# max-andr/joint-cnn-mrf

Hardware: AMD Instinct MI355X
Metric: images/sec (720x480, K=9 joints) part-detector+spatial-model fwd (higher is better)
Workload: dtype f32(fp16x2 spectra, fft); 1 GPU; configs[1]: batch=64/GPU synthetic 480x720x3, part detector + spatial model forward + argmax, fp32; batch_per_gpu=64, global_batch=64, micro_batch=64, use_sm=True, collective=all_gather coords int32 [B,2,9]

## Files before the change

joint-cnn-mrf_amd/csrc/conv_fft.hip:

```cpp
#include <cmath>
#include <cstdlib>
#include <map>
#include <mutex>
#include <utility>
#include <vector>

#include "conv_fft_common.h"

namespace jcm {
namespace cfft {

template <int KS, int NP>
__global__ __launch_bounds__(256) void weight_spectra_split_kernel(const float* __restrict__ w, uint4* __restrict__ Ws, int Cin, int Cout, int CoutP, int ntl, int NY, int NX,
                                                                   int round_bf16, float* __restrict__ wscale) {
  __shared__ cf twy[192][KS - 1], twx[KS];
  const int tid = threadIdx.x;
  const int kx = blockIdx.y;
#pragma unroll 1
  for (int k = tid; k < NY * (KS - 1) + KS; k += 256) {
    const bool isy = k < NY * (KS - 1);
    const int ky = k / (KS - 1), a = isy ? k % (KS - 1) + 1 : k - NY * (KS - 1);
    const int num = isy ? (ky * a) % NY : (kx * a) % NX, den = isy ? NY : NX;
    double sn, cs;
    sincospi(-2.0 * (double)num / (double)den, &sn, &cs);
// ... 115 lines not shown
  }
  block_max_to<256>(m * 1.0001f, wmax, red, threadIdx.x);
}

struct Sizes { int NY, NX; };
static const int kLens[] = {20, 24, 28, 32, 36, 40, 50, 60, 64, 72, 96, 100, 128, 192};
static bool pick(int need, int* n) {
  for (int v : kLens)
    if (v >= need) { *n = v; return true; }
  return false;
}
static int tw_offset(int n) {
  int off = 0;
  for (int v : kLens) {
    if (v == n) return off;
    off += v;
  }
  return -1;
}
static bool sizes_of(int H, int W, int ks, Sizes* s, int circ = 0) {
  if (circ) {
    s->NY = H; s->NX = W;
    return (ks == 9 || ks == 5) && H > 8 && W > 8 && tw_offset(H) >= 0 && tw_offset(W) >= 0;
  }
  return (ks == 9 || ks == 5) && H + ks - 1 <= 192 && W + ks - 1 <= 192 && pick(H + 4, &s->NY) && pick(W + 4, &s->NX);
}
static int pad64(int c) { return (c + CB - 1) / CB * CB; }
static bool fft_reg_on() {
  static const bool on = [] { const char* e = std::getenv("JCM_FFT_REG"); return !e || std::atoi(e) != 0; }();
  return on;
}
static bool fft_tiles_on() {
  static const bool on = [] { const char* e = std::getenv("JCM_FFT_TILES"); return !e || std::atoi(e) != 0; }();
  return on;
}
static int padn(int c, int n) { return (c + n - 1) / n * n; }

int persistent_grid(const void* kernel, int ntiles, int threads, int dyn_lds) {
  static std::mutex mu;
  static std::map<std::pair<const void*, int>, int> cache;
  int dev = 0;
  (void)hipGetDevice(&dev);
  int resident = 0;
  {
    std::lock_guard<std::mutex> lk(mu);
    auto it = cache.find({kernel, dev});
    if (it != cache.end()) resident = it->second;
  }
  if (!resident) {
    int ncu = 256, per_cu = 0;
    (void)hipDeviceGetAttribute(&ncu, hipDeviceAttributeMultiprocessorCount, dev);
    if (hipOccupancyMaxActiveBlocksPerMultiprocessor(&per_cu, kernel, threads, (size_t)dyn_lds) != hipSuccess || per_cu < 1) per_cu = 1;
    resident = ncu * per_cu;
    std::lock_guard<std::mutex> lk(mu);
    cache[{kernel, dev}] = resident;
  }
  return resident < ntiles ? resident : ntiles;
}

static const cf* twiddle_table(int dev) {
  static std::mutex mu;
  static std::map<int, cf*> tabs;
  std::lock_guard<std::mutex> lk(mu);
  auto it = tabs.find(dev);
  if (it != tabs.end()) return it->second;
  std::vector<float> h;
// ... 201 lines not shown
    }
    if (hipError_t ce = cfft_cols_fwd(s.NY, a, np, Tin, Xs, twy, p.NXH, p.MT, sc, st); ce != hipSuccess) return ce;
  }
  if (hipError_t e = hipGetLastError(); e != hipSuccess) return e;
  if (g0 && hipEventRecord(g0, st) != hipSuccess) return hipErrorUnknown;
  const float yshift = sc.t16 ? cgemm_split_y16_shift(a.Cin) : 0.f, yinv = yshift != 0.f ? 1.0f / yshift : 0.f;
  if (hipError_t e = cgemm_split(Xs, a.wp, Yf, np, p.F, a.B, a.Cin, a.Cout, p.ldy, st, yshift); e != hipSuccess) return e;
  if (g1 && hipEventRecord(g1, st) != hipSuccess) return hipErrorUnknown;
  ConvArgs ai = a;
  if (a0.circ) { ai.H = a0.H - 8; ai.W = a0.W - 8; }
  if (!(fft_reg && p.inv_cb == 64 && cfft_cols_inv_reg(s.NY, ai, Yf, T, p.NXH, p.ldy, opad, st, sc.t16_inv, yinv))) cfft_cols_inv(s.NY, ai, Yf, T, twy, p.NXH, p.ldy, opad, st, sc.t16_inv, yinv);
  if (t_next && nx && nx->pool) {
    Sizes sn;
    if (!sizes_of((a.H + 1) / 2, (a.W + 1) / 2, nx->ks_next, &sn) ||
        !cfft_rows_inv_pool_fwd(s.NX, sn.NX, a, T, static_cast<cf*>(t_next), twx, twb + tw_offset(sn.NX), opad, norm, sc, st))
      return hipErrorInvalidValue;
  } else if (t_next && nx && nx->merge) {
    if (sc.t16) {
      float* t16n = reinterpret_cast<float*>(static_cast<char*>(t_next) + align256((size_t)a.B * p.NXH * a.H * a.Cout * 4));
      if (!(fft_reg && cfft_rows_inv_merge_fwd_reg(s.NX, a, *nx->merge, T, static_cast<cf*>(t_next), opad, norm, sc, st, t16n))) return hipErrorInvalidValue;
    } else if (!(fft_reg && cfft_rows_inv_merge_fwd_reg(s.NX, a, *nx->merge, T, static_cast<cf*>(t_next), opad, norm, sc, st)) &&
               !cfft_rows_inv_merge_fwd(s.NX, a, *nx->merge, T, static_cast<cf*>(t_next), twx, opad, norm, sc, st)) {
      return hipErrorInvalidValue;
    }
  } else if (t_next) {
    if (!(fft_reg && cfft_rows_inv_fwd_reg(s.NX, a, T, static_cast<cf*>(t_next), opad, norm, sc, st))) cfft_rows_inv_fwd(s.NX, a, T, static_cast<cf*>(t_next), twx, opad, norm, sc, st);
  } else if (!((ai.rows_mfma & 1) && cfft_rows_inv_mfma(s.NX, ai, out_layout, T, opad, norm, sc, st)) && !(fft_reg && cfft_rows_inv_reg(s.NX, ai, out_layout, T, opad, norm, sc, st))) {
    if (ai.wout_TX > 0) return hipErrorInvalidValue;
    cfft_rows_inv(s.NX, ai, out_layout, T, twx, opad, norm, sc, st);
  }
  return hipGetLastError();
}

size_t conv_fft_xs_bytes(const ConvArgs& a, int ks, int np) {
  Sizes s;
  if (!sizes_of(a.H, a.W, ks, &s, a.circ)) return 0;
  return align256(plan_of(a, s, np).xs_bytes);
}
hipError_t conv_fft_spectra(const ConvArgs& a0, int ks, int np, void* work, void* xs, hipStream_t st, float* tmax, int common) {
  Sizes s;
  if (!conv_fft_supported(a0, ks) || !sizes_of(a0.H, a0.W, ks, &s, a0.circ) || !xs || (np >= 4 && !tmax)) return hipErrorInvalidValue;
  Fp16Scale sc;
  if (np >= 4) { sc.tmax = tmax; sc.hf = (float)a0.H; sc.nb = a0.B; sc.common = common; }
  ConvArgs a = a0;
  a.CoutP = pad64(a.Cout);
  const Plan3 p = plan_of(a, s, np);
  int dev = 0;
  if (hipError_t e = hipGetDevice(&dev); e != hipSuccess) return e;
  const cf* twb = twiddle_table(dev);
  if (!twb) return hipErrorOutOfMemory;
  cf* T = static_cast<cf*>(work);
  if (a.win_map) { if (!cfft_rows_fwd_win_reg(s.NX, a, T, sc.tmax, st)) return hipErrorInvalidValue; }
  else cfft_rows_fwd(s.NX, a, 0, T, twb + tw_offset(s.NX), sc.tmax, st);
  if (hipError_t ce = cfft_cols_fwd(s.NY, a, np, T, xs, twb + tw_offset(s.NY), p.NXH, p.MT, sc, st); ce != hipSuccess) return ce;
  return hipGetLastError();
}
bool conv_fft_geometry(int H, int W, int ks, int B, int Cout, int np, int* NY, int* NX, int* MT, int circ) {
  Sizes s;
  if (!sizes_of(H, W, ks, &s, circ)) return false;
  *NY = s.NY; *NX = s.NX; *MT = cgemm_split_mtile(np, B, Cout);
  return true;
}

}
```

joint-cnn-mrf_amd/csrc/conv_fft_common.h:

```cpp
#pragma once
#include "fft_lds.h"
#include "kernels.h"

namespace jcm {
namespace cfft {
using namespace fftl;
constexpr int CB = 64, NT = 256;
constexpr int kParMax = 512;

template <int N> struct Plan;
template <> struct Plan<192> { static constexpr int R1 = 8, R2 = 8, R3 = 3; };
template <> struct Plan<128> { static constexpr int R1 = 8, R2 = 4, R3 = 4; };
template <> struct Plan<100> { static constexpr int R1 = 4, R2 = 5, R3 = 5; };
template <> struct Plan<96> { static constexpr int R1 = 8, R2 = 12, R3 = 1; };
template <> struct Plan<72> { static constexpr int R1 = 8, R2 = 3, R3 = 3; };
template <> struct Plan<64> { static constexpr int R1 = 8, R2 = 8, R3 = 1; };
template <> struct Plan<60> { static constexpr int R1 = 4, R2 = 15, R3 = 1; };
template <> struct Plan<50> { static constexpr int R1 = 5, R2 = 10, R3 = 1; };
template <> struct Plan<40> { static constexpr int R1 = 8, R2 = 5, R3 = 1; };
template <> struct Plan<36> { static constexpr int R1 = 4, R2 = 3, R3 = 3; };
template <> struct Plan<32> { static constexpr int R1 = 8, R2 = 4, R3 = 1; };
template <> struct Plan<28> { static constexpr int R1 = 4, R2 = 7, R3 = 1; };
template <> struct Plan<24> { static constexpr int R1 = 8, R2 = 3, R3 = 1; };
template <> struct Plan<20> { static constexpr int R1 = 4, R2 = 5, R3 = 1; };
// ... 225 lines not shown
    case 64: CALL(64); break;                    \
    case 72: CALL(72); break;                    \
    case 96: CALL(96); break;                    \
    case 100: CALL(100); break;                  \
    case 128: CALL(128); break;                  \
    default: CALL(192); break;                   \
  }

int persistent_grid(const void* kernel, int ntiles, int threads, int dyn_lds = 0);

void cfft_rows_fwd(int NX, const ConvArgs& a, int layout, cf* T, const cf* tw, float* tmax, hipStream_t st, float* t16 = nullptr);
void cfft_rows_fwd_merge(int NX, const ConvArgs& a, const FftMerge& m, int in_layout, cf* T, const cf* tw, float* tmax, hipStream_t st, float* t16 = nullptr);
hipError_t cfft_cols_fwd(int NY, const ConvArgs& a, int np, const cf* T, void* Xs, const cf* tw, int NXH, int MT, const Fp16Scale& sc, hipStream_t st);
void cfft_cols_inv(int NY, const ConvArgs& a, const cf* Yf, cf* T, const cf* tw, int NXH, int ldy, int pad, hipStream_t st, float* t16 = nullptr, float y16_inv = 0.f);
void cfft_rows_inv(int NX, const ConvArgs& a, int layout, const cf* T, const cf* tw, int pad, float norm, const Fp16Scale& sc, hipStream_t st);
bool cfft_rows_inv_reg(int NX, const ConvArgs& a, int layout, const cf* T, int pad, float norm, const Fp16Scale& sc, hipStream_t st);
bool cfft_rows_inv_fwd_reg(int NX, const ConvArgs& a, const cf* T, cf* Tn, int pad, float norm, const Fp16Scale& sc, hipStream_t st);
bool cfft_rows_fwd_reg(int NX, const ConvArgs& a, int layout, cf* T, float* tmax, hipStream_t st, float* t16);
bool cfft_rows_fwd_win_reg(int NX, const ConvArgs& a, cf* T, float* tmax, hipStream_t st);
bool cfft_rows_fwd_win_reg_supported(int NX, int Cin);
bool cfft_tiles_supported(int NY, int NX, const ConvArgs& a);
bool cfft_rows_fwd_tile_reg(int NY, int NX, const ConvArgs& a, cf* T, float* tmax, hipStream_t st);
bool cfft_rows_inv_pool_tile_reg(int NY, int NX, const ConvArgs& a, const cf* T, cf* Tn, float norm, const Fp16Scale& sc, hipStream_t st);
bool cfft_rows_fwd_merge_reg(int NX, const ConvArgs& a, const FftMerge& m, int in_layout, cf* T, float* tmax, hipStream_t st, float* t16);
bool cfft_cols_inv_reg(int NY, const ConvArgs& a, const cf* Yf, cf* T, int NXH, int ldy, int pad, hipStream_t st, float* t16, float y16_inv = 0.f);
void cfft_rows_inv_fwd(int NX, const ConvArgs& a, const cf* T, cf* Tn, const cf* tw, int pad, float norm, const Fp16Scale& sc, hipStream_t st);
bool cfft_rows_inv_pool_fwd(int NXI, int NXO, const ConvArgs& a, const cf* T, cf* Tn, const cf* twi, const cf* two, int pad, float norm, const Fp16Scale& sc, hipStream_t st);
bool cfft_rows_inv_merge_fwd(int NX, const ConvArgs& a, const FftMerge& m, const cf* T, cf* Tn, const cf* tw, int pad, float norm, const Fp16Scale& sc, hipStream_t st);
bool cfft_rows_inv_merge_fwd_reg(int NX, const ConvArgs& a, const FftMerge& m, const cf* T, cf* Tn, int pad, float norm, const Fp16Scale& sc, hipStream_t st, float* t16n = nullptr);
bool cfft_rows_inv_merge_fwd_reg_supported(int NX, const ConvArgs& a, const FftMerge& m, int pad);
bool cfft_rows_inv_pool_fwd_supported(int NXI, int NXO, int Cout);
bool cfft_rows_inv_mfma(int NX, const ConvArgs& a, int layout, const cf* T, int pad, float norm, const Fp16Scale& sc, hipStream_t st);
bool cfft_rows_inv_merge_fwd_supported(int NX, const ConvArgs& a, const FftMerge& m);
}
}
```

joint-cnn-mrf_amd/csrc/ctx.h:

```cpp
#pragma once
#include "../../include/jcm.h"

#include <map>
#include <mutex>
#include <string>
#include <vector>

#include "kernels.h"

namespace jcm {

struct CallOrder;

int fail(int code, const std::string& msg);

#define HIP_TRY(expr)                                                                                   \
  do {                                                                                                  \
    hipError_t e_ = (expr);                                                                             \
    if (e_ != hipSuccess)                                                                               \
      return ::jcm::fail(JCM_ERR_HIP, std::string(#expr) + ": " + hipGetErrorString(e_));               \
  } while (0)
#define JCM_TRY(expr)          \
  do {                         \
    int r_ = (expr);           \
// ... 27 lines not shown
  void* wp_kxfold = nullptr;
  void* wq1_bf16 = nullptr;
  float* wq1_f32 = nullptr;
  void* wq1_split = nullptr;
  int coutp_bf16 = 0;
  bool thin = false;
  bool thin_bf16 = false;
  const float* bias = nullptr;
  float* scale = nullptr;
  float* shift = nullptr;
};

struct TrainState;
}
struct jcm_ctx;
namespace jcm {
void train_destroy(jcm_ctx* c);
const float* train_param_range(jcm_ctx* c, int64_t off, int64_t n);
const double* train_grad_sumsq(jcm_ctx* c);

}

struct jcm_ctx {
  int device = 0;
  hipStream_t stream = nullptr;
  int precision = JCM_PRECISION_F32;
  int K = 9;
  bool finalized = false;
  int f32_conv = 0;
  int split_min_wgs = 128;
  int sm_algo = 3;
  int conv9_fft = 1;
  int fft_tiles = 1;
  int fft_fuse = 3;
  int fft_single = 1;
  int fft_t16 = 1;
  int fft_rows_mfma = 1;
  int fft_win = 1;
  int bf16_hpool = 1;
  int sm_chunk = 32;
  int micro_batch = 0;
  int call_order = 1;
  int debug_skip = 0;
  std::map<std::string, jcm::Tensor> params;
  std::map<std::string, jcm::ConvLayer> convs;
  std::vector<void*> owned;
  size_t param_bytes = 0;
  bool has_sm = false;
  float* sp_energy = nullptr;
  float* sp_bias = nullptr;
  float* bn_sm_scale = nullptr;
  float* bn_sm_shift = nullptr;
  int* cond = nullptr;
  const float** energy_ptrs = nullptr;
  const float** bias_ptrs = nullptr;
  int* cond0 = nullptr;
  float2* prior_spec_t = nullptr;
  struct FftW { void* p = nullptr; size_t bytes = 0; bool valid = false; float* wscale = nullptr; };
  std::map<std::string, FftW> fft_w;
  double* hist_limits = nullptr;
  jcm::TrainState* train = nullptr;
  char* arena = nullptr;
  size_t arena_cap = 0, arena_off = 0, arena_peak = 0;
  bool dry = false;
  float* act_scale = nullptr;
  float* scale_scratch = nullptr;
// ... 87 lines not shown
```

joint-cnn-mrf_amd/csrc/jcm_api.hip:

```cpp
#include <cmath>
#include <cstdlib>
#include <cstdio>
#include <cstring>

#include <mutex>
#include <vector>

#include "ctx.h"

using namespace jcm;

namespace {
thread_local std::string g_err;
}

namespace jcm {

const char* const kJointNames[10] = {"lsho", "lelb", "lwri", "rsho", "relb", "rwri", "lhip", "rhip", "nose", "torso"};

int fail(int code, const std::string& msg) {
  g_err = msg;
  return code;
}

// ... 219 lines not shown
      jcm_ctx::WordBlock& b = c->fft_blocks[c->fft_block_i];
      if (c->fft_word_i + n <= b.cap) {
        *w = b.p + c->fft_word_i;
        c->fft_word_i += n;
        return JCM_OK;
      }
      ++c->fft_block_i;
      c->fft_word_i = 0;
      continue;
    }
    jcm_ctx::WordBlock b;
    b.cap = n > jcm_ctx::kFftWords ? n : jcm_ctx::kFftWords;
    HIP_TRY(hipMalloc(reinterpret_cast<void**>(&b.p), (size_t)b.cap * sizeof(float)));
    if (hipError_t e = hipMemsetAsync(b.p, 0, (size_t)b.cap * sizeof(float), c->stream); e != hipSuccess) {
      (void)hipFree(b.p);
      return fail(JCM_ERR_HIP, std::string("hipMemsetAsync: ") + hipGetErrorString(e));
    }
    c->fft_blocks.push_back(b);
  }
}
int run_conv_fft(jcm_ctx* c, const ConvLayer* L, const std::string& scope, const void* x, int B, int H, int W, void* out, int in_layout, int out_layout, int circ, FftLink* link) {
  FftLink alone;
  FftLink& k = link ? *link : alone;
  ConvArgs a{};
  a.x = x; a.bias = L->bias; a.scale = L->scale; a.shift = L->shift; a.out = out;
  a.B = B; a.H = H; a.W = W; a.Cin = L->cin; a.Cout = L->cout; a.CoutP = L->cout; a.relu_bn = L->has_bn ? 1 : 0;
  a.circ = circ;
  a.rows_mfma = c->fft_rows_mfma;
  const size_t mark = c->arena_off;
  const int np = fft_np(c);
  a.tiles = c->fft_tiles && k.next.pool && !k.t_in && !k.xs && !k.merge && !k.win_map && !circ && in_layout == 0 &&
            np == 4 && conv_fft_tiles_supported(a, L->ks, k.next.ks_next) ? 1 : 0;
  const int wH = a.tiles ? H / 2 : H, wW = a.tiles ? W / 2 : W;
  void* work = arena_alloc<char>(c, conv_fft_workspace_bytes(a, L->ks, np));
  c->arena_off = mark;
  if (c->dry) return JCM_OK;
  const std::string key = scope + (circ ? "@win" : "@") + std::to_string(wH) + "x" + std::to_string(wW);
  if (!c->fft_w.count(key)) {
    static const size_t cap = [] { const char* e = std::getenv("JCM_FFT_CACHE_GB"); return (size_t)(e ? std::atoi(e) : 64) << 30; }();
    const size_t need = conv_fft_weight_bytes(wH, wW, L->ks, L->cin, L->cout, np, circ);
    size_t held = 0;
    for (auto& kv : c->fft_w) held += kv.second.bytes;
    if (held + need > cap && !c->fft_w.empty()) {
      HIP_TRY(hipStreamSynchronize(c->stream));
      for (auto& kv : c->fft_w) (void)hipFree(kv.second.p);
      c->fft_w.clear();
    }
  }
  jcm_ctx::FftW& fw = c->fft_w[key];
  if (!fw.p) {
    const size_t wb = (conv_fft_weight_bytes(wH, wW, L->ks, L->cin, L->cout, np, circ) + 255) & ~size_t(255);
    fw.bytes = wb + 256;
    if (hipMalloc(&fw.p, fw.bytes) == hipSuccess) {
      fw.wscale = reinterpret_cast<float*>(static_cast<char*>(fw.p) + wb);
    } else {
      const size_t mb = fw.bytes >> 20;
      c->fft_w.erase(key);
      return fail(JCM_ERR_HIP, "out of device memory for the filter spectra of '" + scope + "' (" + std::to_string(mb) + " MB); jcm_set_option(\"conv9_fft\", 0) selects the direct kernels");
    }
  }
  if (!fw.valid) {
    const float* bound_from = nullptr;
    if (np >= 4 && scope.compare(0, 6, "dgrad:") == 0) {
      auto it = c->fft_w.find(key.substr(6));
      if (it != c->fft_w.end() && it->second.valid && it->second.wscale) bound_from = it->second.wscale;
    }
    HIP_TRY(conv_fft_pack_weights(L->w_raw, fw.p, wH, wW, L->ks, L->cin, L->cout, np, c->precision == JCM_PRECISION_BF16, c->stream, fw.wscale, circ, bound_from));
    fw.valid = true;
  }
  a.wp = fw.p;
  hipEvent_t e0 = nullptr, e1 = nullptr, g0 = nullptr, g1 = nullptr;
  JCM_TRY(prof_begin(c, &e0, &e1));
  if (c->profile && (pool_get(c, &g0) != JCM_OK || pool_get(c, &g1) != JCM_OK)) { g0 = g1 = nullptr; }
  if (k.win_map) {
    a.win_map = k.win_map; a.win_B = k.win_B; a.win_H = k.win_H; a.win_W = k.win_W; a.win_TY = k.win_TY; a.win_TX = k.win_TX;
  }
  if (k.win_scatter) {
    a.wout_H = k.win_H; a.wout_W = k.win_W; a.wout_TY = k.win_TY; a.wout_TX = k.win_TX;
  }
  Fp16Scale sc;
  if (np >= 4) {
    sc.tmax = k.tmax_in;
    if ((k.t_in || k.xs_ready) && !sc.tmax) return fail(JCM_ERR_STATE, "conv_fft '" + scope + "': a handed-over tensor without its scale word");
    if (!sc.tmax) JCM_TRY(fft_new_words(c, a.tiles ? 4 * B : B, &sc.tmax));
    if (k.t_next) JCM_TRY(fft_new_words(c, B, &sc.tmax_next));
    sc.winv = fw.wscale + 1;
    sc.common = c->train ? 1 : 0;
    sc.t16 = (np == 5 && c->fft_t16 && in_layout != 0 && out_layout != 0 && !k.xs && (!k.t_in || k.t_in_16) && (!k.t_next || (k.next.merge && !k.t_in))) ? 1 : 0;
  }
  k.tmax = sc.tmax;
  k.tmax_next = sc.tmax_next;
  const hipError_t e = conv_fft_f32(a, L->ks, np, in_layout, out_layout, work, k, g0, g1, c->stream, np >= 4 ? &sc : nullptr);
  if (g0 && g1 && e == hipSuccess) c->prof[scope + "/gemm"].emplace_back(g0, g1);
  else { if (g0) c->event_pool.push_back(g0); if (g1) c->event_pool.push_back(g1); }
  prof_end(c, scope, e0, e1, e == hipSuccess);
  if (e != hipSuccess) return fail(JCM_ERR_HIP, std::string("conv_fft_f32: ") + hipGetErrorString(e));
  return JCM_OK;
}

int run_conv_layer(jcm_ctx* c, const ConvLayer* L, const std::string& scope, int stride, const void* x, int B, int H, int W, int sub,
                   void* out, bool act_bf16, bool out_f32, int in_planar, int out_planar, bool x_u8, FftLink* link, int hpool) {
  const bool fft = stride == 1 && takes_fft(c, L, B, H, W);
  if (!fft && link && !link->empty()) return fail(JCM_ERR_STATE, "layer '" + scope + "' was given a frequency-domain hand-over but does not run in the frequency domain");
  if (hpool && (fft || stride != 1)) return fail(JCM_ERR_STATE, "half pool requested for layer '" + scope + "', which does not run on conv5_strip_bf16_kernel");
  if (stride == 2) {
    if (c->dry) return JCM_OK;
    if (!(L->ks == 5 && L->cin == 3 && L->has_bn))
      return fail(JCM_ERR_ARG, "stride-2 kernel exists for 5x5, Cin=3, BN layers only (" + scope + ")");
    HIP_TRY(conv1_5x5s2(x, L->w_raw, L->bias, L->scale, L->shift, out, act_bf16, B, H, W, sub, L->cout, c->stream, x_u8));
    return JCM_OK;
  }
  if (fft) return run_conv_fft(c, L, scope, x, B, H, W, out, act_bf16 ? (in_planar ? 2 : 1) : 0, (act_bf16 && !out_f32) ? (out_planar ? 2 : 1) : 0, 0, link);
  if (c->dry) return JCM_OK;
  const void* wp = act_bf16 ? L->wp_bf16 : static_cast<const void*>(L->wp);
  if (stride != 1 || !wp) return fail(JCM_ERR_ARG, "no kernel for layer '" + scope + "' with stride " + std::to_string(stride));
  if (!act_bf16 && L->wp_stale) {
    HIP_TRY(pack_weights_f32(L->w_raw, L->wp, L->ks, L->cin, L->cout, L->coutp, c->stream));
    L->wp_stale = false;
  }
  hipEvent_t e0 = nullptr, e1 = nullptr;
  JCM_TRY(prof_begin(c, &e0, &e1));
  const int r = launch_conv_layer(c, L, wp, x, B, H, W, out, act_bf16, out_f32, in_planar, out_planar, hpool);
  prof_end(c, scope, e0, e1, r == JCM_OK);
  return r;
}
// ... 385 lines not shown
  }
  if (k == "debug_skip") {
    h->debug_skip = (int)value;
    return JCM_OK;
  }
  if (k == "call_order") {
    h->call_order = value != 0;
    return JCM_OK;
  }
  if (k == "conv9_fft") {
    h->conv9_fft = value != 0;
    return JCM_OK;
  }
  if (k == "fft_single") {
    if ((value != 0) != (h->fft_single != 0)) {
      HIP_TRY(hipStreamSynchronize(h->stream));
      for (auto& kv : h->fft_w) (void)hipFree(kv.second.p);
      h->fft_w.clear();
    }
    h->fft_single = value != 0;
    return JCM_OK;
  }
  if (k == "fft_windows") {
    h->fft_win = value != 0;
    return JCM_OK;
  }
  if (k == "fft_fuse") {
    if (value < 0 || value > 3) return fail(JCM_ERR_ARG, "fft_fuse must be 0..3 (bit 0: pool hand-over, bit 1: merge hand-over)");
    h->fft_fuse = (int)value;
    return JCM_OK;
  }
  if (k == "fft_tiles") {
    h->fft_tiles = value != 0;
    return JCM_OK;
  }
  if (k == "bf16_hpool") {
    h->bf16_hpool = value != 0;
    return JCM_OK;
  }
  if (k == "fft_rows_mfma") {
    h->fft_rows_mfma = value != 0;
    return JCM_OK;
  }
  if (k == "fft_t16") {
    h->fft_t16 = value != 0;
    return JCM_OK;
  }
  if (k == "sm_chunk") {
    if (value < 1) return fail(JCM_ERR_ARG, "sm_chunk must be >= 1");
    h->sm_chunk = (int)value;
    return JCM_OK;
  }
  if (k == "split_min_wgs") {
    if (value < 0) return fail(JCM_ERR_ARG, "split_min_wgs must be >= 0");
    h->split_min_wgs = (int)value;
    return JCM_OK;
  }
  if (k == "sm_algo") {
    if (value != 1 && value != 3) return fail(JCM_ERR_ARG, "sm_algo must be 3 (every transform in LDS, default) or 1 (direct sliding-window kernel); the rocFFT routes 0 and 2 were removed in round 5");
    h->sm_algo = (int)value;
    return JCM_OK;
  }
  if (h->finalized) return fail(JCM_ERR_STATE, "options must be set before jcm_finalize");
  if (k == "precision") {
    if (value != JCM_PRECISION_F32 && value != JCM_PRECISION_BF16) return fail(JCM_ERR_ARG, "precision must be 0 (f32) or 1 (bf16)");
    h->precision = (int)value;
// ... 479 lines not shown
```

joint-cnn-mrf_amd/csrc/kernels.h:

```cpp
#pragma once
#include <hip/hip_runtime.h>
#include <stdint.h>

#include <atomic>

namespace jcm {

struct LdsAttr {
  std::atomic<uint64_t> done{0};
  hipError_t ensure(const void* fn, int bytes) {
    int dev = 0;
    hipError_t e = hipGetDevice(&dev);
    if (e != hipSuccess) return e;
    const uint64_t bit = 1ull << (dev & 63);
    if (done.load(std::memory_order_acquire) & bit) return hipSuccess;
    e = hipFuncSetAttribute(fn, hipFuncAttributeMaxDynamicSharedMemorySize, bytes);
    if (e == hipSuccess) done.fetch_or(bit, std::memory_order_release);
    return e;
  }
};

struct ConvArgs {
  const void* x;
  const void* wp;
// ... 38 lines not shown
  int nb = 0;
  int common = 0;
  int t16 = 0;
  float* t16_fwd = nullptr;
  float* t16_inv = nullptr;
  int t16_cb = 64;
};
bool conv_fft_supported(const ConvArgs& a, int ks);
size_t conv_fft_weight_bytes(int H, int W, int ks, int Cin, int Cout, int np, int circ = 0);
hipError_t conv_fft_pack_weights(const float* w_hwio, void* wf, int H, int W, int ks, int Cin, int Cout, int np, bool round_bf16, hipStream_t st,
                                 float* wscale = nullptr, int circ = 0,
                                 const float* bound_from = nullptr);
size_t conv_fft_workspace_bytes(const ConvArgs& a, int ks, int np);
struct FftMerge { const void* x2; int H2, W2; const void* x3; int H3, W3; };
struct FftNext { int pool = 0; int ks_next = 0; const FftMerge* merge = nullptr; };
struct FftLink {
  const void* t_in = nullptr;
  bool t_in_16 = false;
  float* tmax_in = nullptr;
  const FftMerge* merge = nullptr;
  void* xs = nullptr;
  bool xs_ready = false;
  const void* win_map = nullptr;
  int win_B = 0, win_H = 0, win_W = 0, win_TY = 0, win_TX = 0;
  void* t_next = nullptr;
  FftNext next;
  bool win_scatter = false;
  float* tmax = nullptr;
  float* tmax_next = nullptr;
  bool empty() const { return !t_in && !merge && !xs && !xs_ready && !win_map && !t_next && !next.pool && !next.merge && !win_scatter; }
};
hipError_t conv_fft_f32(const ConvArgs& a, int ks, int np, int in_layout, int out_layout, void* work, const FftLink& link, hipEvent_t g0, hipEvent_t g1, hipStream_t st,
                        const Fp16Scale* sc = nullptr);
bool conv_fft_win_gather_supported(int win, int Cin);
bool conv_fft_win_scatter_supported(int win, int Cout);
bool conv_fft_pool_fusable(const ConvArgs& a, int ks, int ks_next);
bool conv_fft_tiles_supported(const ConvArgs& a, int ks, int ks_next);
size_t conv_fft_pool_handover_bytes(const ConvArgs& a, int ks_next);
bool conv_fft_merge_fusable(const ConvArgs& a, int ks, int ks_next, const FftMerge& m, bool h16 = false);
size_t conv_fft_xs_bytes(const ConvArgs& a, int ks, int np);
hipError_t conv_fft_spectra(const ConvArgs& a, int ks, int np, void* work, void* xs, hipStream_t st, float* tmax = nullptr, int common = 0);
bool conv_fft_geometry(int H, int W, int ks, int B, int Cout, int np, int* NY, int* NX, int* MT, int circ = 0);

size_t wgrad_fft_scratch_bytes(int NY, int NX, int Cin, int Cout);
hipError_t wgrad_fft(const void* xs, const void* zs, void* scratch, const float* w, float lmbd, float* dw, int ks, int NY, int NX, int B, int MTx, int MTz, int Cin,
                     int ldz, int Cout, hipStream_t st, int np = 3, const float* tmax_x = nullptr, const float* tmax_z = nullptr, int H = 0);
hipError_t pad_channels_f32(const float* in, int ldi, float* out, int ldo, size_t N, hipStream_t st);
hipError_t window_gather_f32(const float* map, float* win, int B, int H, int W, int C, int WS, int TY, int TX, int valid_only, hipStream_t st);
hipError_t window_scatter_f32(const float* val, float* map, int B, int H, int W, int C, int WS, int TY, int TX, hipStream_t st);
bool conv_fft_fusable(const ConvArgs& a, int ks, int ks_next);
size_t conv_fft_handover_bytes(const ConvArgs& a, int ks);

int cgemm_split_mtile(int np, int B, int Cout);
int cgemm_split_ntile(int np, int Cout);
int cgemm_split_parts(int np);
size_t cgemm_split_w_bytes(int np, int F, int Cin, int Cout);
float cgemm_split_y16_shift(int Cin);
hipError_t cgemm_split(const void* xs, const void* ws, void* y, int np, int F, int B, int Cin, int Cout, int ldy, hipStream_t st, float y16_shift = 0.f);

bool conv5_strip_bf16_supported(const ConvArgs& a, int ks);
hipError_t conv5_strip_bf16(const ConvArgs& a, hipStream_t st);

bool conv_kxfold_bf16_supported(const ConvArgs& a, int ks);
size_t conv_kxfold_weight_bytes(int Cin);
hipError_t pack_weights_kxfold(const float* w_hwio, void* wp, int Cin, hipStream_t st);
hipError_t conv_kxfold_bf16(const ConvArgs& a, hipStream_t st);
// ... 147 lines not shown
```

joint-cnn-mrf_amd/engine.py:

```python
import ctypes

import numpy as np
import torch

from . import _lib


def _hm_size(n):
    for _ in range(3):
        n = (n + 1) // 2
    return n


class Engine:

    def __init__(self, device=0, precision='fp32', n_joints=9, stream=None, f32_conv=None, split_min_wgs=None, micro_batch=None, conv9_fft=None, call_order=None, fft_single=None, fft_t16=None, fft_fuse=None, fft_tiles=None):
        if not torch.cuda.is_available():
            raise RuntimeError('joint-cnn-mrf_amd needs an MI355X (gfx950) GPU; torch.cuda.is_available() is False '
                               'and there is no CPU path')
        self._lib = _lib.load()
        self.device = torch.device('cuda', device if isinstance(device, int) else torch.device(device).index or 0)
        self.n_joints = int(n_joints)
        self.precision = precision
        self._stream = stream if stream is not None else torch.cuda.current_stream(self.device)
        h = ctypes.c_void_p()
        _lib.check(self._lib.jcm_create(self.device.index, ctypes.c_void_p(self._stream.cuda_stream), ctypes.byref(h)),
                   'jcm_create')
        self._h = h
        self._finalized = False
        prec = {'fp32': _lib.JCM_PRECISION_F32, 'f32': _lib.JCM_PRECISION_F32, 'bf16': _lib.JCM_PRECISION_BF16}[precision]
        _lib.check(self._lib.jcm_set_option(self._h, b'precision', prec), 'jcm_set_option(precision)')
        _lib.check(self._lib.jcm_set_option(self._h, b'n_joints', self.n_joints), 'jcm_set_option(n_joints)')
        if f32_conv is not None:
            if f32_conv not in ('exact', 'split16'):
                raise ValueError("f32_conv must be 'exact' or 'split16' (the bf16x6 arm 'split' was retired in round 5)")
            _lib.check(self._lib.jcm_set_option(self._h, b'f32_conv', {'exact': 0, 'split16': 2}[f32_conv]), 'jcm_set_option(f32_conv)')
        if micro_batch is not None:
            self.set_micro_batch(micro_batch)
        if conv9_fft is not None:
            self.set_conv9_fft(conv9_fft)
        if fft_single is not None:
            self.set_option('fft_single', int(bool(fft_single)))
        if fft_t16 is not None:
            self.set_option('fft_t16', int(bool(fft_t16)))
        if fft_fuse is not None:
            self.set_option('fft_fuse', int(fft_fuse))
        if fft_tiles is not None:
            self.set_option('fft_tiles', int(bool(fft_tiles)))
        if call_order is not None:
            self.set_option('call_order', int(bool(call_order)))
        if split_min_wgs is not None:
            _lib.check(self._lib.jcm_set_option(self._h, b'split_min_wgs', int(split_min_wgs)), 'jcm_set_option(split_min_wgs)')

    def close(self):
        if getattr(self, '_h', None) is not None and self._h.value:
            self._lib.jcm_destroy(self._h)
            self._h = ctypes.c_void_p()

    def __del__(self):
        try:
            self.close()
        except Exception:
            pass

    def set_tensor(self, name, value):
        if isinstance(value, torch.Tensor):
            t = value.detach().to(torch.float32).contiguous()
            ptr, shape, keep = t.data_ptr(), tuple(t.shape), t
        else:
            a = np.ascontiguousarray(value, dtype=np.float32)
            ptr, shape, keep = a.ctypes.data, a.shape, a
        if len(shape) == 0:
            raise ValueError('scalar parameter %r' % name)
        arr = (ctypes.c_int64 * len(shape))(*shape)
        _lib.check(self._lib.jcm_set_tensor(self._h, name.encode(), ctypes.c_void_p(ptr), arr, len(shape)),
                   'jcm_set_tensor(%s)' % name)
        del keep

    def load_params(self, params, finalize=True):
        for name, value in params.items():
            self.set_tensor(name, value)
# ... 331 lines not shown
```

Before: 7142 images/sec.

## Compute logits 9x9 conv as row-spectrum MFMA GEMM skipping column FFT

Adds a dedicated path for the final 9x9 logits conv (Cout<=16): the input stays in row-FFT spectra and the vertical taps are applied as spatial shifts through fp16 MFMA over 9 dy offsets. This skips the column forward and inverse FFTs, and the output is written straight into a buffer for the inverse row FFT. Weights are prepacked per kx frequency with the horizontal taps folded in. The cost is nine shifted GEMMs in place of one pointwise product, plus another fp16-split precision path and cross-wave reduction overhead.

```diff
diff --git a/joint-cnn-mrf_amd/csrc/conv_fft.hip b/joint-cnn-mrf_amd/csrc/conv_fft.hip
--- a/joint-cnn-mrf_amd/csrc/conv_fft.hip
+++ b/joint-cnn-mrf_amd/csrc/conv_fft.hip
@@ -171,6 +171,10 @@
 }
 static bool fft_tiles_on() {
   static const bool on = [] { const char* e = std::getenv("JCM_FFT_TILES"); return !e || std::atoi(e) != 0; }();
+  return on;
+}
+static bool fft_logits_rows_on() {
+  static const bool on = [] { const char* e = std::getenv("JCM_FFT_LOGITS_ROWS"); return !e || std::atoi(e) != 0; }();
   return on;
 }
 static int padn(int c, int n) { return (c + n - 1) / n * n; }
@@ -438,6 +442,49 @@
   return hipGetLastError();
 }
 
+bool conv_fft_logits_rows_supported(const ConvArgs& a, int ks) {
+  Sizes s;
+  return fft_logits_rows_on() && ks == 9 && !a.circ && !a.tiles && !a.win_map && conv_fft_supported(a, ks) && sizes_of(a.H, a.W, ks, &s) && cfft_logits_rows_supported(s.NX, a);
+}
+size_t conv_fft_logits_weight_bytes(int H, int W, int Cin) {
+  Sizes s;
+  return sizes_of(H, W, 9, &s) ? cfft_logits_rows_operand_bytes(s.NX, Cin) : 0;
+}
+size_t conv_fft_logits_workspace_bytes(const ConvArgs& a) {
+  Sizes s;
+  return sizes_of(a.H, a.W, 9, &s) ? align256((size_t)a.B * a.H * (s.NX / 2 + 1) * CB * sizeof(cf)) : 0;
+}
+hipError_t conv_fft_logits_pack(const float* w_hwio, void* aop, int H, int W, int Cin, int Cout, hipStream_t st, float* wscale) {
+  Sizes s;
+  if (!sizes_of(H, W, 9, &s) || Cin % 16 || Cout > 16 || !wscale) return hipErrorInvalidValue;
+  if (hipError_t e = hipMemsetAsync(wscale, 0, 2 * sizeof(float), st); e != hipSuccess) return e;
+  const size_t pairs = (size_t)Cin * Cout;
+  const dim3 bgrid((unsigned)((pairs + 255) / 256 > 1024 ? 1024 : (pairs + 255) / 256));
+  hipLaunchKernelGGL(weight_bound_kernel<81>, bgrid, dim3(256), 0, st, w_hwio, pairs, 0, wscale);
+  return cfft_logits_rows_pack(s.NX, w_hwio, aop, Cin, Cout, wscale, st);
+}
+hipError_t conv_fft_logits_f32(const ConvArgs& a0, void* work, const FftLink& link, hipEvent_t g0, hipEvent_t g1, hipStream_t st, const Fp16Scale* scp) {
+  Sizes s;
+  if (!conv_fft_logits_rows_supported(a0, 9) || !sizes_of(a0.H, a0.W, 9, &s) || !link.t_in || link.t_in_16 || link.t_next || link.merge || link.xs || link.xs_ready || link.win_scatter ||
+      !scp || !scp->tmax || !scp->winv || scp->common)
+    return hipErrorInvalidValue;
+  ConvArgs a = a0;
+  a.CoutP = pad64(a.Cout);
+  Fp16Scale sc = *scp;
+  sc.hf = 1.f;
+  sc.nb = a.B;
+  int dev = 0;
+  if (hipError_t e = hipGetDevice(&dev); e != hipSuccess) return e;
+  const cf* twb = twiddle_table(dev);
+  if (!twb) return hipErrorOutOfMemory;
+  cf* S = static_cast<cf*>(work);
+  if (g0 && hipEventRecord(g0, st) != hipSuccess) return hipErrorUnknown;
+  if (hipError_t e = cfft_logits_rows(s.NX, a, static_cast<const cf*>(link.t_in), a.wp, sc.tmax, S, st); e != hipSuccess) return e;
+  if (g1 && hipEventRecord(g1, st) != hipSuccess) return hipErrorUnknown;
+  cfft_rows_inv(s.NX, a, 0, S, twb + tw_offset(s.NX), 4, 1.0f / (float)s.NX, sc, st);
+  return hipGetLastError();
+}
+
 size_t conv_fft_xs_bytes(const ConvArgs& a, int ks, int np) {
   Sizes s;
   if (!sizes_of(a.H, a.W, ks, &s, a.circ)) return 0;
diff --git a/joint-cnn-mrf_amd/csrc/conv_fft_common.h b/joint-cnn-mrf_amd/csrc/conv_fft_common.h
--- a/joint-cnn-mrf_amd/csrc/conv_fft_common.h
+++ b/joint-cnn-mrf_amd/csrc/conv_fft_common.h
@@ -281,5 +281,9 @@
 bool cfft_rows_inv_pool_fwd_supported(int NXI, int NXO, int Cout);
 bool cfft_rows_inv_mfma(int NX, const ConvArgs& a, int layout, const cf* T, int pad, float norm, const Fp16Scale& sc, hipStream_t st);
 bool cfft_rows_inv_merge_fwd_supported(int NX, const ConvArgs& a, const FftMerge& m);
-}
-}
+bool cfft_logits_rows_supported(int NX, const ConvArgs& a);
+size_t cfft_logits_rows_operand_bytes(int NX, int Cin);
+hipError_t cfft_logits_rows_pack(int NX, const float* w_hwio, void* aop, int Cin, int Cout, float* wscale, hipStream_t st);
+hipError_t cfft_logits_rows(int NX, const ConvArgs& a, const cf* T, const void* aop, const float* tmax, cf* S, hipStream_t st);
+}
+}
diff --git a/joint-cnn-mrf_amd/csrc/conv_fft_logits.hip b/joint-cnn-mrf_amd/csrc/conv_fft_logits.hip
--- /dev/null
+++ b/joint-cnn-mrf_amd/csrc/conv_fft_logits.hip
@@ -0,0 +1,171 @@
+#include "conv_fft_common.h"
+
+namespace jcm {
+namespace cfft {
+
+constexpr int kLrWaves = 8, kLrRows = 72, kLrUnits = 8;
+constexpr int kLrLds = kLrWaves * kLrRows * kLrUnits * 16;
+typedef _Float16 f16x8 __attribute__((ext_vector_type(8)));
+typedef float f32x4 __attribute__((ext_vector_type(4)));
+
+__device__ __forceinline__ int lr_slot(int r, int u) { return r * kLrUnits + (u ^ ((r >> 1) & 7)); }
+
+__global__ __launch_bounds__(256) void logits_rows_operand_kernel(const float* __restrict__ w, uint4* __restrict__ Aop, int Cin, int Cout, int NX, float* __restrict__ wscale) {
+  __shared__ cf twx[9];
+  const int kx = blockIdx.y, KC = Cin >> 4;
+  if (threadIdx.x < 9) {
+    double sn, cs;
+    sincospi(-2.0 * (double)((kx * (int)threadIdx.x) % NX) / (double)NX, &sn, &cs);
+    twx[threadIdx.x] = cf{(float)cs, (float)sn};
+  }
+  __syncthreads();
+  int ex = 0;
+  const float bound = wscale[0];
+  if (bound > 0.f && bound < 3.0e38f) (void)frexpf(bound, &ex);
+  const float wmul = ldexpf(1.f, 14 - ex);
+  if (blockIdx.x == 0 && blockIdx.y == 0 && threadIdx.x == 0) wscale[1] = ldexpf(1.f, ex - 14);
+  const int e = blockIdx.x * 256 + threadIdx.x;
+  if (e >= 9 * KC * 64) return;
+  const int lane = e & 63, c = (e >> 6) % KC, dy = (e >> 6) / KC;
+  const int j = lane & 15, g = lane >> 4, ch0 = c * 16 + (g & 1) * 8;
+  cf a[8];
+#pragma unroll
+  for (int i = 0; i < 8; ++i) a[i] = cf{0.f, 0.f};
+  if (j < Cout) {
+#pragma unroll
+    for (int b = 0; b < 9; ++b) {
+      const float* tap = w + ((size_t)(dy * 9 + (8 - b)) * Cin + ch0) * Cout + j;
+      const cf tw = twx[b];
+#pragma unroll
+      for (int i = 0; i < 8; ++i) a[i] = sfma(tap[(size_t)i * Cout], tw, a[i]);
+    }
+  }
+  float vr[8], vi[8];
+#pragma unroll
+  for (int i = 0; i < 8; ++i) {
+    vr[i] = g < 2 ? a[i].x : -a[i].y;
+    vi[i] = g < 2 ? a[i].y : a[i].x;
+  }
+  uint4 u[2];
+  uint4* dst = Aop + ((((size_t)kx * 9 + dy) * KC + c) * 4) * 64 + lane;
+  split8h(vr, wmul, u);
+  dst[0] = u[0]; dst[64] = u[1];
+  split8h(vi, wmul, u);
+  dst[128] = u[0]; dst[192] = u[1];
+}
+
+__global__ __launch_bounds__(512) __attribute__((amdgpu_waves_per_eu(4, 4))) void logits_rows_kernel(const float4* __restrict__ T, const uint4* __restrict__ Aop,
+                                                                                                       const float* __restrict__ tmax, cf* __restrict__ S, int B, int H, int KC,
+                                                                                                       int NXH, int per) {
+  extern __shared__ __attribute__((aligned(16))) char lr_smem[];
+  const int xcd = blockIdx.x & 7, slot = blockIdx.x >> 3, item = xcd * per + slot;
+  if (slot >= per || item >= NXH * B) return;
+  const int kx = item / B, b = item - kx * B;
+  const int tid = threadIdx.x, wave = tid >> 6, lane = tid & 63;
+  uint4* wl = reinterpret_cast<uint4*>(lr_smem) + wave * (kLrRows * kLrUnits);
+  for (int i = lane; i < kLrRows * kLrUnits; i += 64) wl[i] = make_uint4(0u, 0u, 0u, 0u);
+  const float scale = fp16_scale(tmax[b], 1.f);
+  f32x4 sr[4], si[4];
+#pragma unroll
+  for (int m = 0; m < 4; ++m) { sr[m] = f32x4{0.f, 0.f, 0.f, 0.f}; si[m] = f32x4{0.f, 0.f, 0.f, 0.f}; }
+  const int y0 = lane >> 1, y1 = 32 + (lane >> 1), hh = lane & 1;
+  const bool in0 = y0 < H, in1 = y1 < H;
+  float4 pre[2][4];
+  auto fetch = [&](int c) __attribute__((always_inline)) {
+    const float4* src = T + (((size_t)kx * KC + c) * B + b) * H * 8 + hh * 4;
+#pragma unroll
+    for (int q = 0; q < 4; ++q) {
+      pre[0][q] = in0 ? src[(size_t)y0 * 8 + q] : make_float4(0.f, 0.f, 0.f, 0.f);
+      pre[1][q] = in1 ? src[(size_t)y1 * 8 + q] : make_float4(0.f, 0.f, 0.f, 0.f);
+    }
+  };
+  auto stash = [&](int i, int y) __attribute__((always_inline)) {
+    float re[8], im[8];
+#pragma unroll
+    for (int q = 0; q < 4; ++q) { re[2 * q] = pre[i][q].x; im[2 * q] = pre[i][q].y; re[2 * q + 1] = pre[i][q].z; im[2 * q + 1] = pre[i][q].w; }
+    uint4 ur[2], ui[2];
+    split8h(re, scale, ur);
+    split8h(im, scale, ui);
+    const int r = y + 4;
+    wl[lr_slot(r, hh)] = ur[0]; wl[lr_slot(r, 2 + hh)] = ui[0];
+    wl[lr_slot(r, 4 + hh)] = ur[1]; wl[lr_slot(r, 6 + hh)] = ui[1];
+  };
+  const int g = lane >> 4, rl = lane & 15;
+  if (wave < KC) fetch(wave);
+  for (int c = wave; c < KC; c += kLrWaves) {
+    if (in0) stash(0, y0);
+    if (in1) stash(1, y1);
+    if (c + kLrWaves < KC) fetch(c + kLrWaves);
+    __builtin_amdgcn_fence(__ATOMIC_RELEASE, "wavefront");
+    __builtin_amdgcn_wave_barrier();
+    __builtin_amdgcn_fence(__ATOMIC_ACQUIRE, "wavefront");
+    const uint4* bp = Aop + (((size_t)kx * 9 * KC + c) * 4) * 64 + lane;
+#pragma unroll 3
+    for (int dy = 0; dy < 9; ++dy) {
+      const uint4* bq = bp + (size_t)dy * KC * 256;
+      const f16x8 br0 = __builtin_bit_cast(f16x8, bq[0]), br1 = __builtin_bit_cast(f16x8, bq[64]);
+      const f16x8 bi0 = __builtin_bit_cast(f16x8, bq[128]), bi1 = __builtin_bit_cast(f16x8, bq[192]);
+#pragma unroll
+      for (int m = 0; m < 4; ++m) {
+        const int r = m * 16 + rl + dy;
+        const f16x8 a0 = __builtin_bit_cast(f16x8, wl[lr_slot(r, g)]), a1 = __builtin_bit_cast(f16x8, wl[lr_slot(r, 4 + g)]);
+        sr[m] = __builtin_amdgcn_mfma_f32_16x16x32_f16(a0, br1, sr[m], 0, 0, 0);
+        si[m] = __builtin_amdgcn_mfma_f32_16x16x32_f16(a0, bi1, si[m], 0, 0, 0);
+        sr[m] = __builtin_amdgcn_mfma_f32_16x16x32_f16(a1, br0, sr[m], 0, 0, 0);
+        si[m] = __builtin_amdgcn_mfma_f32_16x16x32_f16(a1, bi0, si[m], 0, 0, 0);
+        sr[m] = __builtin_amdgcn_mfma_f32_16x16x32_f16(a0, br0, sr[m], 0, 0, 0);
+        si[m] = __builtin_amdgcn_mfma_f32_16x16x32_f16(a0, bi0, si[m], 0, 0, 0);
+      }
+    }
+    __builtin_amdgcn_fence(__ATOMIC_RELEASE, "wavefront");
+    __builtin_amdgcn_wave_barrier();
+    __builtin_amdgcn_fence(__ATOMIC_ACQUIRE, "wavefront");
+  }
+  __syncthreads();
+  float* red = reinterpret_cast<float*>(lr_smem);
+#pragma unroll
+  for (int m = 0; m < 4; ++m)
+#pragma unroll
+    for (int i = 0; i < 4; ++i) {
+      red[(wave * 32 + m * 4 + i) * 64 + lane] = sr[m][i];
+      red[(wave * 32 + 16 + m * 4 + i) * 64 + lane] = si[m][i];
+    }
+  __syncthreads();
+  cf* Sb = S + ((size_t)b * H * NXH + kx) * 64;
+#pragma unroll
+  for (int q = 0; q < 2; ++q) {
+    const int pi = tid + 512 * q, lo = pi & 63, mi = pi >> 6;
+    float re = 0.f, im = 0.f;
+#pragma unroll
+    for (int wv = 0; wv < kLrWaves; ++wv) {
+      re += red[(wv * 32 + mi) * 64 + lo];
+      im += red[(wv * 32 + 16 + mi) * 64 + lo];
+    }
+    const int row = (mi >> 2) * 16 + (lo >> 4) * 4 + (mi & 3);
+    if (row < H) Sb[(size_t)row * NXH * 64 + (lo & 15)] = cf{re, im};
+  }
+  for (int e = tid; e < H * 24; e += 512) {
+    const int row = e / 24, q = e - row * 24;
+    *reinterpret_cast<float4*>(Sb + (size_t)row * NXH * 64 + 16 + 2 * q) = make_float4(0.f, 0.f, 0.f, 0.f);
+  }
+}
+
+bool cfft_logits_rows_supported(int NX, const ConvArgs& a) { return NX == 96 && a.H >= 1 && a.H <= 64 && a.Cin % 16 == 0 && a.Cout >= 1 && a.Cout <= 16 && a.B >= 1; }
+size_t cfft_logits_rows_operand_bytes(int NX, int Cin) { return (size_t)(NX / 2 + 1) * 9 * (Cin / 16) * 4 * 64 * sizeof(uint4); }
+hipError_t cfft_logits_rows_pack(int NX, const float* w_hwio, void* aop, int Cin, int Cout, float* wscale, hipStream_t st) {
+  const dim3 grid((unsigned)((9 * (Cin / 16) * 64 + 255) / 256), (unsigned)(NX / 2 + 1));
+  hipLaunchKernelGGL(logits_rows_operand_kernel, grid, dim3(256), 0, st, w_hwio, static_cast<uint4*>(aop), Cin, Cout, NX, wscale);
+  return hipGetLastError();
+}
+hipError_t cfft_logits_rows(int NX, const ConvArgs& a, const cf* T, const void* aop, const float* tmax, cf* S, hipStream_t st) {
+  if (!cfft_logits_rows_supported(NX, a)) return hipErrorInvalidValue;
+  static LdsAttr attr;
+  if (hipError_t e = attr.ensure(reinterpret_cast<const void*>(logits_rows_kernel), kLrLds); e != hipSuccess) return e;
+  const int NXH = NX / 2 + 1, items = NXH * a.B, per = (items + 7) / 8;
+  hipLaunchKernelGGL(logits_rows_kernel, dim3((unsigned)(per * 8)), dim3(512), kLrLds, st, reinterpret_cast<const float4*>(T), static_cast<const uint4*>(aop), tmax, S, a.B, a.H,
+                     a.Cin / 16, NXH, per);
+  return hipGetLastError();
+}
+
+}
+}
diff --git a/joint-cnn-mrf_amd/csrc/ctx.h b/joint-cnn-mrf_amd/csrc/ctx.h
--- a/joint-cnn-mrf_amd/csrc/ctx.h
+++ b/joint-cnn-mrf_amd/csrc/ctx.h
@@ -83,6 +83,7 @@
   int sm_algo = 3;
   int conv9_fft = 1;
   int fft_tiles = 1;
+  int fft_logits_rows = 1;
   int fft_fuse = 3;
   int fft_single = 1;
   int fft_t16 = 1;
diff --git a/joint-cnn-mrf_amd/csrc/jcm_api.hip b/joint-cnn-mrf_amd/csrc/jcm_api.hip
--- a/joint-cnn-mrf_amd/csrc/jcm_api.hip
+++ b/joint-cnn-mrf_amd/csrc/jcm_api.hip
@@ -275,13 +275,16 @@
   a.tiles = c->fft_tiles && k.next.pool && !k.t_in && !k.xs && !k.merge && !k.win_map && !circ && in_layout == 0 &&
             np == 4 && conv_fft_tiles_supported(a, L->ks, k.next.ks_next) ? 1 : 0;
   const int wH = a.tiles ? H / 2 : H, wW = a.tiles ? W / 2 : W;
-  void* work = arena_alloc<char>(c, conv_fft_workspace_bytes(a, L->ks, np));
+  const bool lrows = c->fft_logits_rows && !c->train && np == 4 && k.t_in && !k.t_in_16 && !k.t_next && !k.next.pool && !k.next.merge && !k.xs && !k.xs_ready && !k.merge &&
+                     !k.win_map && !k.win_scatter && !circ && in_layout == 0 && out_layout == 0 && conv_fft_logits_rows_supported(a, L->ks);
+  void* work = arena_alloc<char>(c, lrows ? conv_fft_logits_workspace_bytes(a) : conv_fft_workspace_bytes(a, L->ks, np));
   c->arena_off = mark;
   if (c->dry) return JCM_OK;
-  const std::string key = scope + (circ ? "@win" : "@") + std::to_string(wH) + "x" + std::to_string(wW);
+  const std::string key = scope + (circ ? "@win" : lrows ? "@rows" : "@") + std::to_string(wH) + "x" + std::to_string(wW);
+  const size_t wbytes = lrows ? conv_fft_logits_weight_bytes(wH, wW, L->cin) : conv_fft_weight_bytes(wH, wW, L->ks, L->cin, L->cout, np, circ);
   if (!c->fft_w.count(key)) {
     static const size_t cap = [] { const char* e = std::getenv("JCM_FFT_CACHE_GB"); return (size_t)(e ? std::atoi(e) : 64) << 30; }();
-    const size_t need = conv_fft_weight_bytes(wH, wW, L->ks, L->cin, L->cout, np, circ);
+    const size_t need = wbytes;
     size_t held = 0;
     for (auto& kv : c->fft_w) held += kv.second.bytes;
     if (held + need > cap && !c->fft_w.empty()) {
@@ -292,7 +295,7 @@
   }
   jcm_ctx::FftW& fw = c->fft_w[key];
   if (!fw.p) {
-    const size_t wb = (conv_fft_weight_bytes(wH, wW, L->ks, L->cin, L->cout, np, circ) + 255) & ~size_t(255);
+    const size_t wb = (wbytes + 255) & ~size_t(255);
     fw.bytes = wb + 256;
     if (hipMalloc(&fw.p, fw.bytes) == hipSuccess) {
       fw.wscale = reinterpret_cast<float*>(static_cast<char*>(fw.p) + wb);
@@ -308,7 +311,8 @@
       auto it = c->fft_w.find(key.substr(6));
       if (it != c->fft_w.end() && it->second.valid && it->second.wscale) bound_from = it->second.wscale;
     }
-    HIP_TRY(conv_fft_pack_weights(L->w_raw, fw.p, wH, wW, L->ks, L->cin, L->cout, np, c->precision == JCM_PRECISION_BF16, c->stream, fw.wscale, circ, bound_from));
+    if (lrows) HIP_TRY(conv_fft_logits_pack(L->w_raw, fw.p, wH, wW, L->cin, L->cout, c->stream, fw.wscale));
+    else HIP_TRY(conv_fft_pack_weights(L->w_raw, fw.p, wH, wW, L->ks, L->cin, L->cout, np, c->precision == JCM_PRECISION_BF16, c->stream, fw.wscale, circ, bound_from));
     fw.valid = true;
   }
   a.wp = fw.p;
@@ -333,7 +337,8 @@
   }
   k.tmax = sc.tmax;
   k.tmax_next = sc.tmax_next;
-  const hipError_t e = conv_fft_f32(a, L->ks, np, in_layout, out_layout, work, k, g0, g1, c->stream, np >= 4 ? &sc : nullptr);
+  const hipError_t e = lrows ? conv_fft_logits_f32(a, work, k, g0, g1, c->stream, &sc)
+                             : conv_fft_f32(a, L->ks, np, in_layout, out_layout, work, k, g0, g1, c->stream, np >= 4 ? &sc : nullptr);
   if (g0 && g1 && e == hipSuccess) c->prof[scope + "/gemm"].emplace_back(g0, g1);
   else { if (g0) c->event_pool.push_back(g0); if (g1) c->event_pool.push_back(g1); }
   prof_end(c, scope, e0, e1, e == hipSuccess);
@@ -785,6 +790,10 @@
   }
   if (k == "fft_tiles") {
     h->fft_tiles = value != 0;
+    return JCM_OK;
+  }
+  if (k == "fft_logits_rows") {
+    h->fft_logits_rows = value != 0;
     return JCM_OK;
   }
   if (k == "bf16_hpool") {
diff --git a/joint-cnn-mrf_amd/csrc/kernels.h b/joint-cnn-mrf_amd/csrc/kernels.h
--- a/joint-cnn-mrf_amd/csrc/kernels.h
+++ b/joint-cnn-mrf_amd/csrc/kernels.h
@@ -94,6 +94,11 @@
 };
 hipError_t conv_fft_f32(const ConvArgs& a, int ks, int np, int in_layout, int out_layout, void* work, const FftLink& link, hipEvent_t g0, hipEvent_t g1, hipStream_t st,
                         const Fp16Scale* sc = nullptr);
+bool conv_fft_logits_rows_supported(const ConvArgs& a, int ks);
+size_t conv_fft_logits_weight_bytes(int H, int W, int Cin);
+size_t conv_fft_logits_workspace_bytes(const ConvArgs& a);
+hipError_t conv_fft_logits_pack(const float* w_hwio, void* aop, int H, int W, int Cin, int Cout, hipStream_t st, float* wscale);
+hipError_t conv_fft_logits_f32(const ConvArgs& a, void* work, const FftLink& link, hipEvent_t g0, hipEvent_t g1, hipStream_t st, const Fp16Scale* sc);
 bool conv_fft_win_gather_supported(int win, int Cin);
 bool conv_fft_win_scatter_supported(int win, int Cout);
 bool conv_fft_pool_fusable(const ConvArgs& a, int ks, int ks_next);
diff --git a/joint-cnn-mrf_amd/engine.py b/joint-cnn-mrf_amd/engine.py
--- a/joint-cnn-mrf_amd/engine.py
+++ b/joint-cnn-mrf_amd/engine.py
@@ -14,7 +14,7 @@
 
 class Engine:
 
-    def __init__(self, device=0, precision='fp32', n_joints=9, stream=None, f32_conv=None, split_min_wgs=None, micro_batch=None, conv9_fft=None, call_order=None, fft_single=None, fft_t16=None, fft_fuse=None, fft_tiles=None):
+    def __init__(self, device=0, precision='fp32', n_joints=9, stream=None, f32_conv=None, split_min_wgs=None, micro_batch=None, conv9_fft=None, call_order=None, fft_single=None, fft_t16=None, fft_fuse=None, fft_tiles=None, fft_logits_rows=None):
         if not torch.cuda.is_available():
             raise RuntimeError('joint-cnn-mrf_amd needs an MI355X (gfx950) GPU; torch.cuda.is_available() is False '
                                'and there is no CPU path')
@@ -47,6 +47,8 @@
             self.set_option('fft_fuse', int(fft_fuse))
         if fft_tiles is not None:
             self.set_option('fft_tiles', int(bool(fft_tiles)))
+        if fft_logits_rows is not None:
+            self.set_option('fft_logits_rows', int(bool(fft_logits_rows)))
         if call_order is not None:
             self.set_option('call_order', int(bool(call_order)))
         if split_min_wgs is not None:
```

Result: faster. 7257 images/sec (median of 6 runs) (+1.6%).
